# facebookresearch/vector_db_id_compression

Measured on AMD Instinct MI355X. Metric: IDs encoded+decoded / sec (ROC/ANS, bit-exact vs codec.cpp), higher is better.
Workload: dtype u64

## Files before the change

vector_db_id_compression_amd/csrc/roc_u2.h:

```cpp
#pragma once
#include "roc_u.h"
#include "roc_u2_geom.h"

namespace vidc {
namespace dev {

template <int UB>
__device__ __forceinline__ uint32_t u2_word_of(uint32_t x) {
    using U = U2Geom<UB>;
    return (((x >> U::ESH) ^ (U::NE - 1u)) << U::GSH) | ((x >> 6) & (U::G - 1u));
}

__device__ __forceinline__ uint32_t u2_dec_word_of(uint32_t x) { return x >> 6; }

typedef uint4 U2Div;

template <int UB>
__device__ __forceinline__ void u2_build_counts(const uint64_t *bm, uint32_t &E1, v32u &ra, v32u &rb) {
    using U = U2Geom<UB>;
    const uint32_t lane = lane_id();
    uint32_t running = 0;
    E1 = 0;
#pragma unroll
    for (int L1 = 63; L1 >= 0; L1--) {
// ... 137 lines not shown
#else
#define U2P(i) ""
#define U2P_OPERANDS
#endif
#define U2_DIV \
    "v_mul_hi_u32 v36, s58, v7\n"                       \
    "v_mad_u64_u32 v[38:39], s[78:79], s58, v8, v[36:37]\n" \
    "v_mad_u64_u32 v[42:43], s[78:79], s59, v7, v[38:39]\n" \
    "v_mov_b32 v40, v43\n" \
    "v_mad_u64_u32 v[46:47], s[78:79], s59, v8, v[40:41]\n"
#define U2_DIV_REM \
    "v_mul_lo_u32 v48, v46, v9\n" \
    "v_sub_u32 v48, s58, v48\n"
#define U2_INSTALL \
    "v_mov_b32 v7, v54\n v_mov_b32 v8, v55\n v_mov_b32 v10, v56\n v_mov_b32 v11, v57\n" \
    "v_sub_u32 v9, s85, v2\n" \
    "v_max_i32 v9, 1, v9\n" \
    "v_sub_u32 v29, 0, v9\n" \
    "s_sub_u32 s68, s85, 63\n" \
    "v_sub_u32 v58, s68, v2\n" \
    "v_max_i32 v58, 0, v58\n" \
    "v_lshlrev_b32 v58, 4, v58\n" \
    "global_load_dwordx4 v[54:57], v58, s[94:95]\n"
#define U2_ENC_ENTRY \
    "v_sub_u32 v58, s85, v2\n" \
    "v_max_i32 v58, 0, v58\n" \
    "v_lshlrev_b32 v58, 4, v58\n" \
    "global_load_dwordx4 v[54:57], v58, s[94:95]\n" \
    "s_waitcnt vmcnt(0)\n" \
    U2_INSTALL U2_DIV U2_DIV_REM \
    "s_mov_b32 s69, 0\n" \
    "s_min_u32 s70, s86, 63\n"

#define U2_ENC_TOP "1:\n" U2_ENC_TOP_NL
#define U2_ENC_TOP_NL \
    U2P(130) U2P(131) \
    "v_lshrrev_b32_e64 v14, 16, s40\n"                  \
    "v_bfe_u32 v15, s40, 0, 16\n"                       \
    "v_add_u32 v16, v48, v14\n"                         \
    "v_mad_u32_u24 v16, v15, s41, v16\n"                \
    "v_mul_hi_u32 v17, v16, v10\n"                      \
    "v_mad_i32_i24 v18, v17, v29, v16\n"                \
    "v_sub_u32 v19, v18, v9\n" \
    "v_min_u32 v52, v18, v19\n"                         \
    "v_ashrrev_i32 v27, 31, v19\n"                      \
    "v_add3_u32 v20, v17, v27, 1\n"                     \
    "v_readlane_b32 s42, v52, s69\n"                    \
    "v_add_co_u32_e64 v50, s[78:79], v46, v20\n"        \
    "v_addc_co_u32_e64 v51, s[78:79], 0, v47, s[78:79]\n" \
    "v_mov_b32 v12, s42\n" U2P(132) \
    "v_cmp_le_u32 vcc, v4, v12\n"                       \
    "v_lshlrev_b64 v[22:23], s40, 1\n"                  \
    "v_bfi_b32 v24, v22, 0, s66\n" \
    "v_readlane_b32 s50, v50, s69\n" \
    "v_readlane_b32 s51, v51, s69\n" \
    U2P(133) \
    "v_bfi_b32 v25, v23, 0, s67\n" \
    "v_mov_b32 v26, s65\n" \
    "ds_write_b64 v26, v[24:25]\n" \
    "s_ff1_i32_b64 s43, vcc\n" \
    "s_set_gpr_idx_on s43, gpr_idx(SRC0)\n" \
    "v_mov_b32 v13, v64\n"                              \
    "s_set_gpr_idx_off\n" U2P(134) \
    "s_and_b32 m0, s60, 63\n"                           \
    "s_cmp_ge_u32 s51, s73\n" \
    "v_writelane_b32 v5, s50, m0\n" \
// ... 73 lines not shown
    "s_sub_u32 s68, s60, s61\n"                         \
    "s_cmp_ge_u32 s68, 48\n" \
    "s_cselect_b32 s71, 0, s71\n"
#define U2_ENC_BOT(ORDER, LSHR) U2_ENC_BOT_T(ORDER, LSHR, U2_RING_CHECK, "s_cbranch_scc1 1b\n")
#define U2_ENC_BOT_T(ORDER, LSHR, RING, TAIL) \
    "v_mbcnt_lo_u32_b32 v49, s66, 0\n" \
    "v_mbcnt_hi_u32_b32 v49, s67, v49\n" \
    "v_cmp_eq_u32 vcc, v49, v12\n"                      \
    "v_sub_u32 v48, s58, v48\n"                         \
    "s_and_b64 s[82:83], vcc, s[66:67]\n" \
    "s_ff1_i32_b64 s48, s[82:83]\n" \
    "s_or_b32 s40, s46, s48\n"                          U2P(140) \
    "s_mov_b32 m0, s62\n" \
    "s_and_b32 s68, s40, 0xffff\n" \
    "s_or_b32 s68, s68, s54\n" \
    "v_writelane_b32 v5, s68, m0\n"                     \
    ORDER U2P(141) \
    "s_set_gpr_idx_on s43, gpr_idx(DST)\n" \
    "v_mov_b32 v64, v13\n" \
    "s_set_gpr_idx_off\n" U2P(142) \
    LSHR                                                \
    "s_cselect_b32 s71, s70, 0\n" \
    "s_cmp_ge_u32 s59, 0x7ff80000\n" \
    "s_cselect_b32 s71, 0, s71\n" \
    RING \
    "s_add_u32 s69, s69, 1\n" U2P(143) \
    "s_cmp_lt_u32 s69, s71\n" \
    TAIL
#define U2_ENC_ORDER \
    "s_mov_b32 m0, s69\n" \
    "s_lshr_b64 s[98:99], s[58:59], 31\n"              \
    "v_writelane_b32 v6, s40, m0\n"

#define U2_ENC_TOP_D \
    U2P(130) U2P(131) \
    "v_lshrrev_b32_e64 v14, 16, s40\n"                  \
    "v_bfe_u32 v15, s40, 0, 16\n"                       \
    "v_add_u32 v16, v48, v14\n"                         \
    "v_mad_u32_u24 v16, v15, s41, v16\n"                \
    "v_mul_hi_u32 v17, v16, v10\n"                      \
    "v_mad_i32_i24 v18, v17, v29, v16\n"                \
    "v_sub_u32 v19, v18, v9\n" \
    "v_min_u32 v52, v18, v19\n"                         \
    "v_ashrrev_i32 v27, 31, v19\n"                      \
    "v_add3_u32 v20, v17, v27, 1\n"                     \
    "v_readlane_b32 s42, v52, s69\n"                    U2P(132) \
    "v_cmp_ge_u32_e64 s[82:83], s42, v4\n"              \
    "v_add_co_u32_e64 v50, s[78:79], v46, v20\n"        \
    "v_addc_co_u32_e64 v51, s[78:79], 0, v47, s[78:79]\n" \
    "v_readlane_b32 s50, v50, s69\n" \
    "v_readlane_b32 s51, v51, s69\n" \
    U2P(133) \
    "s_ff1_i32_b64 s43, s[82:83]\n" \
    "s_set_gpr_idx_on s43, gpr_idx(SRC0)\n" \
    "v_mov_b32 v13, v64\n"                              \
    "s_set_gpr_idx_off\n" U2P(134) \
    "s_and_b32 m0, s60, 63\n"                           \
    "s_cmp_ge_u32 s51, s73\n" \
    "v_writelane_b32 v5, s50, m0\n" \
    "s_cselect_b32 s52, s51, s50\n" \
    "s_cselect_b32 s53, 0, s51\n" \
    "s_addc_u32 s60, s60, 0\n" \
    "s_lshl_b64 s[54:55], s[52:53], s76\n" \
    "s_and_b32 s62, s60, 63\n"                          \
    "s_cmp_ge_u32 s55, s74\n" \
    "s_cselect_b32 s41, 0, s75\n" \
    "s_cselect_b32 s56, s55, s54\n" \
    "s_cselect_b32 s57, 0, s55\n" \
    "s_addc_u32 s60, s60, 0\n" \
    "s_lshl_b64 s[58:59], s[56:57], s77\n"              U2P(135) \
    "v_readlane_b32 s49, v4, s43\n" \
    "v_add_u32 v27, s49, v13\n"                         \
    "v_cmp_ge_u32 vcc, s42, v27\n"                      \
    "v_mul_hi_u32 v36, s58, v7\n"                       \
    "s_ff1_i32_b64 s44, vcc\n" \
    "s_lshl_b32 s45, s43, 6\n" \
    "s_or_b32 s45, s45, s44\n" U2P(136)
#define U2_ENC_MID_D \
    "v_lshl_add_u32 v28, s45, 5, v3\n" \
    "v_lshlrev_b32_e64 v26, 2, s45\n" \
    "ds_read_u16 v30, v28 offset:2\n" \
    "ds_read_b32 v31, v26 offset:16\n"                  \
    "v_readlane_b32 s63, v27, s44\n"                    \
    "v_cndmask_b32_e64 v59, -1, 0, vcc\n"               \
    "v_add_u32 v13, v13, v59\n"                         \
    "v_cndmask_b32_e64 v59, -1, 0, s[82:83]\n"          \
    "v_add_u32 v4, v4, v59\n"                           U2P(137) \
    "s_sub_u32 s42, s42, s63\n"                         \
    "v_cmp_lt_u32_e64 s[82:83], s42, v60\n"             U2P(138) \
    "v_mad_u64_u32 v[38:39], s[78:79], s58, v8, v[36:37]\n" \
    "v_mad_u64_u32 v[42:43], s[78:79], s59, v7, v[38:39]\n" \
    "v_mov_b32 v40, v43\n" \
    "v_mad_u64_u32 v[46:47], s[78:79], s59, v8, v[40:41]\n" \
    "s_waitcnt lgkmcnt(0)\n" U2P(139)
#define U2_ENC_BOT_D(ORDER, LSHR, RING, TAIL) \
    "v_add_u32 v32, v30, v31\n"                         \
    "v_cndmask_b32_e64 v61, v62, v28, s[82:83]\n"       \
    "v_readlane_b32 s40, v32, s42\n"                    \
    "ds_write_b16 v61, v30\n"                           \
    "v_mul_lo_u32 v48, v46, v9\n"                       \
    "v_sub_u32 v48, s58, v48\n"                         U2P(140) \
    "s_mov_b32 m0, s62\n" \
    "s_and_b32 s68, s40, 0xffff\n" \
    "s_or_b32 s68, s68, s54\n" \
    "v_writelane_b32 v5, s68, m0\n"                     \
    ORDER U2P(141) \
    "s_set_gpr_idx_on s43, gpr_idx(DST)\n" \
    "v_mov_b32 v64, v13\n" \
    "s_set_gpr_idx_off\n" U2P(142) \
    LSHR                                                \
    "s_cselect_b32 s71, s70, 0\n" \
    "s_cmp_ge_u32 s59, 0x7ff80000\n" \
    "s_cselect_b32 s71, 0, s71\n" \
    RING \
    "s_add_u32 s69, s69, 1\n" U2P(143) \
    "s_cmp_lt_u32 s69, s71\n" \
    TAIL

#define U2_ORDER_FLUSH \
    "v_cmp_gt_u32 vcc, s72, v2\n" \
    "v_add_u32 v58, s87, v2\n" \
    "v_lshlrev_b32 v58, 2, v58\n" \
    "s_and_saveexec_b64 s[96:97], vcc\n" \
    "global_store_dword v58, v6, s[88:89]\n" \
    "s_mov_b64 exec, s[96:97]\n" \
    "s_add_u32 s87, s87, s72\n"

#define U2_ENC_OUTER(FLUSH) \
    "s_lshr_b64 s[98:99], s[58:59], 31\n"              \
    "s_cselect_b32 s99, 0, 1\n" \
    "s_cmp_ge_u32 s59, 0x7ff80000\n" \
    "s_cselect_b32 s99, 1, s99\n" \
    "s_sub_u32 s68, s60, s61\n" \
    "s_cmp_lt_u32 s68, 48\n"                            \
    "s_cbranch_scc1 3f\n" \
    "v_subrev_u32 v27, s61, v2\n"                       \
    "v_and_b32 v27, 63, v27\n" \
    "v_add_u32 v58, s61, v27\n" \
    "v_cmp_gt_u32 vcc, 32, v27\n" \
    "v_cmp_gt_u32 s[96:97], s92, v58\n" \
    "v_lshlrev_b32 v58, 2, v58\n" \
    "s_and_b64 vcc, vcc, s[96:97]\n" \
    "s_and_saveexec_b64 s[96:97], vcc\n" \
    "global_store_dword v58, v5, s[90:91]\n" \
    "s_mov_b64 exec, s[96:97]\n" \
    "s_add_u32 s61, s61, 32\n" \
    "s_cmp_gt_u32 s61, s92\n" \
    "s_cselect_b32 s68, 1, 0\n" \
    "s_or_b32 s93, s93, s68\n" \
    "3:\n" \
// ... 104 lines not shown
    const uint32_t p0 = P < 16u ? P : 16u, p1 = P > 16u ? P - 16u : 0u;
    WStack st;
    {
        const uint64_t ao = rfl64(arena_at(a, l));
        ws_init_empty(st, a.arena + ao, rfl((uint32_t)(arena_at(a, l + 1) - ao)), a.mt, VIDC_MT_TABLE);
    }
    uint64_t head = VIDC_RANS_L;
    uint32_t obuf = 0, obase = 0;
    uint32_t *order = WANT_ORDER ? a.perm + off : nullptr;
    const uint32_t T0 = 0x80000000u >> p0, T1 = 0x80000000u >> p1, MULN = 1u << p1;
    const uint32_t l3off = dense ? 2u * lane + (U2Dense::SLOT_OFF - 2u) : U::G == 4u ? (lane & 3u) * 8u : 0u;
    const uint32_t rmlane = lane - 1u < 15u ? lane : 0u, strip = U2Dense::STRIP_OFF + 4u * lane;

#ifdef U2_PROF
    uint32_t prof[14] = {0, 0, 0, 0, 0, 0, 0, 0, 0, 0, 0, 0, 0, 0};
#endif
#ifdef U2_PROF2
    uint64_t prof2[8] = {0, 0, 0, 0, 0, 0, 0, 0};
    prof2[2] = __builtin_readcyclecounter();
#endif
    uint32_t nmax = n;
    while (nmax) {
        if (st.sp - st.lo >= U2_RING_ROOM) ws_spill32(st);
        if (nmax < 3u || u2_needs_generic(head)) {
            const uint32_t x = dense ? u2d_slow_step(head, st, nmax, E1, ra, rb, smem, p0, p1)
                                     : u2_slow_step<UB>(head, st, nmax, E1, ra, rb, bm, p0, p1);
            if (WANT_ORDER) {
                if (lane == 0) order[obase] = x;
                obase++;
            }
            nmax--;
            continue;
        }
        uint32_t s_x = 0, s_mul = 0, s_t = 0, s_waddr = U::BITMAP_BYTES, s_D0 = rfl(nmax), s_left = rfl(nmax - 2u);
        uint64_t s_w = 0, s_B = rfl64(head);
        uint64_t z0 = 0, z1 = 0, z2 = 0;
        uint64_t qh = 0;
        uint32_t rr = 0;
        st.sp = rfl(st.sp);
        st.lo = rfl(st.lo);
        st.err = rfl(st.err);
        obase = rfl(obase);
#ifdef U2_PROF2
        const uint64_t tp0 = __builtin_readcyclecounter();
#endif
#define U2_ENC_ASM(BODY)                                                                                                  \
        asm volatile(BODY                                                                                                 \
            : "+{v4}"(E1), "+{v5}"(st.win), "+{v6}"(obuf), "+{v[64:95]}"(ra), "+{v[96:127]}"(rb),                          \
              "+{v[46:47]}"(qh), "+{v48}"(rr), "+{s40}"(s_x), "+{s41}"(s_mul), "+{s[58:59]}"(s_B), "+{s60}"(st.sp),          \
              "+{s61}"(st.lo), "+{s65}"(s_waddr), "+{s[66:67]}"(s_w), "+{s69}"(s_t), "+{s85}"(s_D0), "+{s86}"(s_left),       \
              "+{s87}"(obase), "+{s93}"(st.err), "+{v[20:21]}"(z0), "+{v[36:37]}"(z1), "+{v[40:41]}"(z2) U2P_OPERANDS       \
            : "{v2}"(lane), "{v3}"(l3off), "{s73}"(T0), "{s74}"(T1), "{s75}"(MULN), "{s76}"(p0), "{s77}"(p1),                \
              "{s[88:89]}"(order), "{s[90:91]}"(st.mem), "{s92}"(st.cap), "{s[94:95]}"(dtab), "{v60}"(rmlane), "{v62}"(strip) \
            : "memory", "vcc", "scc", "v7", "v8", "v9", "v10", "v11", "v12", "v13", "v14", "v15", "v16", "v17", "v18", "v19",  \
              "v22", "v23", "v24", "v25", "v26", "v27", "v28", "v29", "v30", "v31", "v32", "v33", "v34", "v35", "v38", "v39",\
              "v42", "v43", "v44", "v45", "v49", "v50", "v51", "v52", "v54", "v55", "v56", "v57", "v58", "v59", "v61",              \
              "s42", "s43", "s44", "s45", "s46", "s47", "s48", "s49", "s50", "s51", "s52", "s53", "s54", "s55", "s56", "s57",\
              "s62", "s63", "s64", "s68", "s70", "s71", "s72", "s78", "s79", "s80", "s81", "s82", "s83", "s84", "s96",       \
              "s97", "s98", "s99")
        if (dense) {
#define U2_STEP_D(ORDER, LSHR) U2_ENC_TOP_D U2_ENC_MID_D U2_ENC_BOT_D(ORDER, LSHR, "", "s_cbranch_scc0 7f\n")
#define U2_LAST_D(ORDER, LSHR) U2_ENC_TOP_D U2_ENC_MID_D U2_ENC_BOT_D(ORDER, LSHR, U2_RING_CHECK, "s_cbranch_scc1 1b\n")
            if (WANT_ORDER) U2_ENC_ASM(U2_ENC_ENTRY "1:\n" U2_STEP_D(U2_ENC_ORDER, "") U2_STEP_D(U2_ENC_ORDER, "") U2_STEP_D(U2_ENC_ORDER, "") U2_STEP_D(U2_ENC_ORDER, "") U2_STEP_D(U2_ENC_ORDER, "") U2_STEP_D(U2_ENC_ORDER, "") U2_STEP_D(U2_ENC_ORDER, "")
                                       U2_LAST_D(U2_ENC_ORDER, "") "7:\n" U2_ENC_OUTER(U2_ORDER_FLUSH));
            else U2_ENC_ASM(U2_ENC_ENTRY "1:\n" U2_STEP_D("", "s_lshr_b64 s[98:99], s[58:59], 31\n") U2_STEP_D("", "s_lshr_b64 s[98:99], s[58:59], 31\n") U2_STEP_D("", "s_lshr_b64 s[98:99], s[58:59], 31\n")
                            U2_LAST_D("", "s_lshr_b64 s[98:99], s[58:59], 31\n") "7:\n" U2_ENC_OUTER(""));
#undef U2_STEP_D
#undef U2_LAST_D
        } else if (U::G == 4u) {
#define U2_STEP_X(ORDER, LSHR) U2_ENC_TOP_NL U2_ENC_MID_G4 U2_ENC_SLICE1_G4 U2_ENC_L3_G4 U2_ENC_BOT_T(ORDER, LSHR, "", "s_cbranch_scc0 7f\n")
            if (WANT_ORDER) U2_ENC_ASM(U2_ENC_ENTRY "1:\n" U2_STEP_X(U2_ENC_ORDER, "") U2_STEP_X(U2_ENC_ORDER, "") U2_STEP_X(U2_ENC_ORDER, "") U2_STEP_X(U2_ENC_ORDER, "") U2_STEP_X(U2_ENC_ORDER, "") U2_STEP_X(U2_ENC_ORDER, "") U2_STEP_X(U2_ENC_ORDER, "")
                                       U2_ENC_TOP_NL U2_ENC_MID_G4 U2_ENC_SLICE1_G4 U2_ENC_L3_G4 U2_ENC_BOT(U2_ENC_ORDER, "") "7:\n" U2_ENC_OUTER(U2_ORDER_FLUSH));
            else U2_ENC_ASM(U2_ENC_ENTRY "1:\n" U2_STEP_X("", "s_lshr_b64 s[98:99], s[58:59], 31\n") U2_STEP_X("", "s_lshr_b64 s[98:99], s[58:59], 31\n") U2_STEP_X("", "s_lshr_b64 s[98:99], s[58:59], 31\n")
                            U2_ENC_TOP_NL U2_ENC_MID_G4 U2_ENC_SLICE1_G4 U2_ENC_L3_G4 U2_ENC_BOT("", "s_lshr_b64 s[98:99], s[58:59], 31\n") "7:\n" U2_ENC_OUTER(""));
#undef U2_STEP_X
        } else {
#define U2_STEP_X1(ORDER, LSHR) U2_ENC_TOP_NL U2_ENC_MID_G1 U2_ENC_SLICE1("6") U2_ENC_L3_G1 U2_ENC_BOT_T(ORDER, LSHR, "", "s_cbranch_scc0 7f\n")
            if (WANT_ORDER) U2_ENC_ASM(U2_ENC_ENTRY "1:\n" U2_STEP_X1(U2_ENC_ORDER, "") U2_STEP_X1(U2_ENC_ORDER, "") U2_STEP_X1(U2_ENC_ORDER, "") U2_STEP_X1(U2_ENC_ORDER, "") U2_STEP_X1(U2_ENC_ORDER, "") U2_STEP_X1(U2_ENC_ORDER, "") U2_STEP_X1(U2_ENC_ORDER, "")
                                       U2_ENC_TOP_NL U2_ENC_MID_G1 U2_ENC_SLICE1("6") U2_ENC_L3_G1 U2_ENC_BOT(U2_ENC_ORDER, "") "7:\n" U2_ENC_OUTER(U2_ORDER_FLUSH));
            else U2_ENC_ASM(U2_ENC_ENTRY "1:\n" U2_STEP_X1("", "s_lshr_b64 s[98:99], s[58:59], 31\n") U2_STEP_X1("", "s_lshr_b64 s[98:99], s[58:59], 31\n") U2_STEP_X1("", "s_lshr_b64 s[98:99], s[58:59], 31\n")
                            U2_ENC_TOP_NL U2_ENC_MID_G1 U2_ENC_SLICE1("6") U2_ENC_L3_G1 U2_ENC_BOT("", "s_lshr_b64 s[98:99], s[58:59], 31\n") "7:\n" U2_ENC_OUTER(""));
#undef U2_STEP_X1
        }
#undef U2_ENC_ASM
#ifdef U2_PROF2
        prof2[0] += __builtin_readcyclecounter() - tp0;
        prof2[1] += 1;
        prof2[4] += s_t == 63u;
        prof2[5] += st.sp - st.lo >= 62u;
        prof2[6] += u2_needs_generic(s_B);
        prof2[7] += s_t;
#endif
        head = s_B + (uint64_t)((s_x & 0xffffu) * s_mul + (s_x >> 16));
        if (!dense) bm[s_waddr >> 3] = s_w & ~(1ull << (s_x & 63u));
        ws_window(st);
        if (__builtin_expect((head >> 63) != 0ull, 0)) {
            ws_prepare(st);
            ans_u_push(head, st, 0u, 0u);
            ans_u_push(head, st, 0u, 0u);
// ... 298 lines not shown
#define U2_DEC_TOP_L(LA, LB, LC, LD)                    \
    U2PD(130) U2PD(131) \
    "s_and_b32 s46, s58, s73\n"                         \
    "s_lshr_b64 s[58:59], s[58:59], s77\n" \
    "s_lshr_b64 s[98:99], s[58:59], 31\n"              \
    "s_cbranch_scc0 " LA "f\n"                          \
    LB ":\n" \
    "s_and_b32 s40, s58, s74\n"                         \
    "s_lshr_b64 s[58:59], s[58:59], s76\n" \
    "s_lshr_b64 s[98:99], s[58:59], 31\n" \
    "s_cbranch_scc0 " LC "f\n" \
    LD ":\n" \
    "s_pack_ll_b32_b16 s40, s40, s46\n"                 U2PD(132)
#define U2_DEC_IDX_G4 \
    "s_lshr_b32 s45, s40, 8\n"                          \
    "v_lshl_add_u32 v28, s45, 5, v3\n" \
    "v_lshlrev_b32_e64 v29, 2, s45\n"                   \
    "ds_read_b64 v[30:31], v28\n" \
    "ds_read_b32 v29, v29\n"                            \
    "s_bfe_u32 s47, s40, 0x20006\n"                     \
    "s_lshr_b32 s65, s40, 5\n"                          U2PD(133)
#define U2_DEC_IDX_G1 \
    "s_lshr_b32 s45, s40, 6\n" \
    "v_lshl_add_u32 v28, s45, 3, v3\n" \
    "v_lshlrev_b32_e64 v29, 2, s45\n" \
    "ds_read_b64 v[30:31], v28\n" \
    "ds_read_b32 v29, v29\n" \
    "s_lshr_b32 s65, s40, 5\n" U2PD(133)
#define U2_DEC_AFTER_RANK \
    "v_writelane_b32 v6, s40, m0\n"                     \
    "v_ashrrev_i32 v58, 31, v58\n" \
    "v_sub_u32 v4, v4, v58\n"                           U2PD(142)
#ifndef U2_DEC_STEP
#define U2_DEC_STEP 3
#endif
#define U2_DEC_TOP_P(LA, LB) \
    U2PD(130) U2PD(131) \
    "s_lshr_b64 s[98:99], s[58:59], s56\n"             \
    "s_cbranch_scc0 " LA "f\n" \
    "s_and_b32 s46, s58, s73\n"                         \
    "s_bfe_u32 s40, s58, s57\n"                         \
    "s_lshr_b64 s[58:59], s[58:59], s63\n"              \
    "s_lshr_b64 s[98:99], s[58:59], 31\n"              \
    "s_cselect_b32 s59, s59, s58\n"                     \
    "s_cselect_b32 s58, s58, s41\n" \
    "s_addc_u32 s60, s60, -1\n"                         \
    LB ":\n" \
    "s_pack_ll_b32_b16 s40, s40, s46\n"                 U2PD(132)
#define U2_DEC_SIDE_P(LA, LB) \
    LA ":\n"                                            \
    "s_and_b32 s46, s58, s73\n" \
    "s_lshr_b64 s[58:59], s[58:59], s77\n" \
    "s_sub_u32 s60, s60, 1\n" \
    "s_mov_b32 s59, s58\n" \
    "s_mov_b32 s58, s41\n" \
    "s_and_b32 s40, s58, s74\n" \
    "s_lshr_b64 s[58:59], s[58:59], s76\n" \
    "s_branch " LB "b\n"
#if U2_DEC_STEP & 2
#define U2_DEC_W_IDX "s_sub_u32 s42, s60, 1\n"
#define U2_DEC_W_LOAD "v_readlane_b32 s41, v5, s42\n"
#else
#define U2_DEC_W_IDX ""
#define U2_DEC_W_LOAD ""
#endif
#if U2_DEC_STEP & 1
#define U2_DEC_BFM ""
// ... 77 lines not shown
    "ds_read_u16 v29, v29\n"                            \
    "s_lshr_b32 s65, s40, 5\n"                          U2PD(133)
#define U2_DEC_MID_W \
    "s_lshr_b32 s43, s45, 8\n"                          \
    "s_and_b32 s44, s45, 255\n"                         \
    U2_DEC_BFM \
    "s_and_b32 m0, s60, 63\n" U2PD(134) \
    "v_readlane_b32 s62, v10, s69\n"                    \
    "v_readlane_b32 s49, v4, s43\n"                     \
    "v_lshl_add_u32 v38, s43, 9, v11\n"                 \
    "v_lshl_add_u32 v39, s44, 4, v3\n"                  \
    "v_med3_i32 v39, v39, 0, 63\n" \
    "v_writelane_b32 v5, s58, m0\n"                     \
    "v_lshlrev_b64 v[34:35], v39, s[54:55]\n"           \
    "v_and_b32 v35, 0x7fffffff, v35\n"                  U2PD(135) \
    "s_cmp_ge_u32 s59, s62\n" \
    "s_cselect_b32 s50, s59, s58\n" \
    "s_cselect_b32 s51, 0, s59\n" \
    "s_addc_u32 s60, s60, 0\n" U2PD(136) \
    U2_DEC_W_IDX \
    "s_mul_i32 s52, s50, s75\n"                         \
    "s_mul_hi_u32 s53, s50, s75\n" \
    "s_mul_i32 s68, s51, s75\n" \
    "s_add_u32 s53, s53, s68\n" \
    "s_mov_b32 m0, s69\n" U2PD(137)
#define U2_DEC_RANK_W \
    U2_DEC_RANK_1W("32") \
    U2_DEC_W_LOAD                                       \
    U2_DEC_INS_ADDR \
    "v_lshlrev_b32 v27, s40, v12\n"                     \
    "v_writelane_b32 v6, s40, m0\n"                     \
    "ds_or_b32 v26, v27\n"                              \
    "ds_add_u64 v38, v[34:35]\n"                        U2PD(141)
#define U2_DEC_BOT_T_U(RLO, RSPAN)                      \
    "s_sub_u32 s68, s60, s61\n"                         \
    "s_add_u32 s68, s68, " RLO "\n" \
    "s_add_u32 s69, s69, 1\n" \
    "s_add_u32 s75, s75, 1\n" \
    "s_add_u32 s58, s52, s64\n"                         \
    "s_addc_u32 s59, s53, 0\n" \
    "s_cmp_gt_u32 s68, " RSPAN "\n" \
    "s_cselect_b32 s71, 0, s70\n" \
    "s_lshr_b64 s[98:99], s[58:59], 31\n"              \
    "s_cselect_b32 s71, s71, 0\n" U2PD(143) \
    "s_cmp_lt_u32 s69, s71\n"
#define U2_DEC_BOT_NR_U \
    "s_add_u32 s69, s69, 1\n" \
    "s_add_u32 s75, s75, 1\n" \
    "s_add_u32 s58, s52, s64\n"                         \
    "s_addc_u32 s59, s53, 0\n" \
    "s_lshr_b64 s[98:99], s[58:59], 31\n"              \
    "s_cselect_b32 s71, s70, 0\n" U2PD(143) \
    "s_cmp_lt_u32 s69, s71\n"
#if U2_DEC_STEP & 2
#define U2_DEC_TOP_U(LA, LB, LC, LD) U2_DEC_TOP_P(LA, LB)
#define U2_DEC_SIDE_U(LA, LB, LC, LD) U2_DEC_SIDE_P(LA, LB)
#define U2_DEC_ENTRY_U U2_DEC_ENTRY U2_DEC_W_IDX U2_DEC_W_LOAD
#define U2_DEC_OUTER_U(RLO, RSPAN) U2_DEC_OUTER_TR(RLO, RSPAN, U2_DEC_W_IDX U2_DEC_W_LOAD)
#else
#define U2_DEC_TOP_U(LA, LB, LC, LD) U2_DEC_TOP_L(LA, LB, LC, LD)
#define U2_DEC_SIDE_U(LA, LB, LC, LD) U2_DEC_SIDE(LA, LB, LC, LD)
#define U2_DEC_ENTRY_U U2_DEC_ENTRY
#define U2_DEC_OUTER_U(RLO, RSPAN) U2_DEC_OUTER_T(RLO, RSPAN)
#endif
#define U2_DEC_STEP_U(IDX, MID, RANK, LA, LB, LC, LD) U2_DEC_TOP_U(LA, LB, LC, LD) IDX MID RANK U2_DEC_BOT_NR_U "s_cbranch_scc0 2f\n"
#define U2_DEC_LOOP8_U(IDX, MID, RANK) \
// ... 182 lines not shown
    const uint32_t M1 = (1u << p1) - 1u, M0 = (1u << p0) - 1u;
    const uint32_t pop_thr = 31u + p1, pop_bfe = (p0 << 16) | p1, pop_sh = p1 + p0;
    uint64_t *out = a.out + ooff;
    wave_sync();
#ifdef U2_PROF
    uint32_t prof[14] = {0, 0, 0, 0, 0, 0, 0, 0, 0, 0, 0, 0, 0, 0};
#endif

#ifdef U2_PROF2
    uint32_t dbg[4] = {0, 0, 0, 0};
#define U2_DBG(k) dbg[k]++
#else
#define U2_DBG(k)
#endif
    uint32_t i = 0;
    constexpr uint32_t RING_LO = U2_DEC_RING_LO, RING_HI = U2_DEC_RING_HI;
    while (i < n) {
        {
            const uint32_t res = st.sp - st.lo;
            if (res > 56u) ws_spill32(st);
            else if (res < 22u && st.lo != 0u) ws_refill32(st);
        }
        if (lt_2p31(head) || st.sp - st.lo < RING_LO || st.sp - st.lo > RING_HI) {
            U2_DBG(0);
            uint32_t x;
            if constexpr (WORD) x = u2w_slow_dec_step(head, st, i + 1u, E1, smem, p0, p1);
            else x = u2_slow_dec_step<UB>(head, st, i + 1u, E1, rows, bm, p0, p1);
            if (lane == 0) out[n - 1u - i] = (uint64_t)x;
            i++;
            continue;
        }
        U2_DBG(1);
        uint32_t s_t = 0, s_N0 = rfl(i + 1u), s_left = rfl(n - i), s_oidx = rfl(n - 1u - i);
        uint64_t s_h = rfl64(head), oring = 0;
        st.sp = rfl(st.sp);
        st.lo = rfl(st.lo);
#define U2_DEC_IN_W "{v12}"(ins_bit), "{s[54:55]}"(field_ones),
#define U2_DEC_ASM(BODY, ...)                                                                                             \
        asm volatile(BODY                                                                                                 \
            : "+{v4}"(E1), "+{v5}"(st.win), "+{v[6:7]}"(oring),                                                           \
              "+{s[58:59]}"(s_h), "+{s60}"(st.sp), "+{s69}"(s_t), "+{s85}"(s_N0), "+{s86}"(s_left), "+{s87}"(s_oidx)        \
              U2P_OPERANDS                                                                                                 \
            : __VA_ARGS__ "{v2}"(lane), "{v3}"(l3off), "{v8}"(ins_mul), "{v9}"(ins_add), "{v11}"(row_lane), "{s61}"(st.lo), \
              "{s73}"(M1), "{s74}"(M0), "{s76}"(p0), "{s77}"(p1), "{s[88:89]}"(out), "{s[94:95]}"(dtab),                    \
              "{s56}"(pop_thr), "{s57}"(pop_bfe), "{s63}"(pop_sh)                                                            \
            : "memory", "vcc", "scc", "v10", "v26", "v27", "v28", "v29", "v30", "v31", "v32", "v33", "v34", "v35", "v36",     \
              "v37", "v38", "v39", "v54", "v55", "v56", "v57", "v58", "s40", "s41", "s42", "s43", "s44", "s45", "s46", "s47", \
              "s49", "s50", "s51", "s52", "s53", "s62", "s64", "s65", "s66", "s67", "s68", "s70", "s71", "s72", "s75", "s96", \
              "s97", "s98", "s99" U2PD_CLOBBERS)
        if constexpr (WORD) U2_DEC_ASM(U2_DEC_ENTRY_U U2_DEC_LOOP8_U(U2_DEC_IDX_W, U2_DEC_MID_W, U2_DEC_RANK_W) U2_DEC_OUTER_U("-18", "35"), U2_DEC_IN_W);
        else if (U::G == 4u) U2_DEC_ASM(U2_DEC_ENTRY_U U2_DEC_LOOP8_U(U2_DEC_IDX_G4, U2_DEC_MID_U, U2_DEC_RANK_U_G4) U2_DEC_OUTER_U("-18", "35"));
        else U2_DEC_ASM(U2_DEC_ENTRY_U U2_DEC_LOOP8_U(U2_DEC_IDX_G1, U2_DEC_MID_U1, U2_DEC_RANK_U_G1) U2_DEC_OUTER_U("-18", "35"));
#undef U2_DEC_ASM
#undef U2_DEC_IN_W
        head = s_h;
        ws_window(st);
        if (__builtin_expect(lt_2p31(head), 0)) {
            ws_prepare(st);
            head = (uint64_t)ws_pop(st) | (head << 32);
        }
        i = s_N0 + s_t - 1u;
    }
    uint32_t bits = 0;
    for (uint32_t w = lane; w < U::BITMAP_BYTES / 8u; w += 64) bits += popc64(bm[w]);
#pragma unroll
    for (int o = 32; o > 0; o >>= 1) bits += (uint32_t)__shfl_xor((int)bits, o, 64);
#ifdef U2_PROF2
    if (lane == 0) { a.slots[0] = dbg[0]; a.slots[1] = dbg[1]; a.slots[2] = rfl(bits); a.slots[3] = n; }
#endif
#ifdef U2_PROF
    if (lane == 0)
        for (int q = 0; q < 14; q++) a.slots[q] = prof[q];
#endif
    if (rfl(bits) != n) {
        wave_sync();
        roc_decode_u_body<UB>(a, smem);
        return;
    }
    if (lane == 0) {
        const bool clean = (head == VIDC_RANS_L) && (st.sp == st.draws - draws0);
        a.end_state[l] = clean ? 0u : 1u;
        a.status[l] = st.err ? ((st.err & 1u) ? VIDC_ST_OVERFLOW : VIDC_ST_MT) : VIDC_ST_OK;
    }
// ... 318 lines not shown
```

Baseline: 61.44 million.

## Add classified fast-path renormalization for dense encode and word decode loops

Restructures the dense encoder step so the common case, where the head needs no renormalization (checked by one shift against 63-P), does a single combined shift and skips both slice compare/select sequences. Renormalizing steps branch to out-of-line side blocks. In the word decoder it adds a classified loop (enabled by raising U2_DEC_STEP to 7) that decodes both slices with one combined shift and branches out only for the rare refill or spill cases, limiting block length where the classification stays valid. A host-side reference header models the classified math for validation. The cost is extra branches and code size, plus a risk to bit-exactness in the rare paths.

Result: faster. 65.52 million (median of 6 runs) (+6.6%).

```diff
diff --git a/vector_db_id_compression_amd/csrc/roc_u2.h b/vector_db_id_compression_amd/csrc/roc_u2.h
--- a/vector_db_id_compression_amd/csrc/roc_u2.h
+++ b/vector_db_id_compression_amd/csrc/roc_u2.h
@@ -193,6 +193,9 @@
     "s_mov_b32 s69, 0\n" \
     "s_min_u32 s70, s86, 63\n"
 
+#ifndef U2_ENC_STEP
+#define U2_ENC_STEP 1
+#endif
 #define U2_ENC_TOP "1:\n" U2_ENC_TOP_NL
 #define U2_ENC_TOP_NL \
     U2P(130) U2P(131) \
@@ -332,7 +335,7 @@
     "s_lshr_b64 s[98:99], s[58:59], 31\n"              \
     "v_writelane_b32 v6, s40, m0\n"
 
-#define U2_ENC_TOP_D \
+#define U2_ENC_TOP_D_A \
     U2P(130) U2P(131) \
     "v_lshrrev_b32_e64 v14, 16, s40\n"                  \
     "v_bfe_u32 v15, s40, 0, 16\n"                       \
@@ -354,7 +357,8 @@
     "s_ff1_i32_b64 s43, s[82:83]\n" \
     "s_set_gpr_idx_on s43, gpr_idx(SRC0)\n" \
     "v_mov_b32 v13, v64\n"                              \
-    "s_set_gpr_idx_off\n" U2P(134) \
+    "s_set_gpr_idx_off\n" U2P(134)
+#define U2_ENC_SLICES_D(MULSEL) \
     "s_and_b32 m0, s60, 63\n"                           \
     "s_cmp_ge_u32 s51, s73\n" \
     "v_writelane_b32 v5, s50, m0\n" \
@@ -364,11 +368,12 @@
     "s_lshl_b64 s[54:55], s[52:53], s76\n" \
     "s_and_b32 s62, s60, 63\n"                          \
     "s_cmp_ge_u32 s55, s74\n" \
-    "s_cselect_b32 s41, 0, s75\n" \
+    MULSEL \
     "s_cselect_b32 s56, s55, s54\n" \
     "s_cselect_b32 s57, 0, s55\n" \
     "s_addc_u32 s60, s60, 0\n" \
-    "s_lshl_b64 s[58:59], s[56:57], s77\n"              U2P(135) \
+    "s_lshl_b64 s[58:59], s[56:57], s77\n"
+#define U2_ENC_TOP_D_B \
     "v_readlane_b32 s49, v4, s43\n" \
     "v_add_u32 v27, s49, v13\n"                         \
     "v_cmp_ge_u32 vcc, s42, v27\n"                      \
@@ -376,6 +381,7 @@
     "s_ff1_i32_b64 s44, vcc\n" \
     "s_lshl_b32 s45, s43, 6\n" \
     "s_or_b32 s45, s45, s44\n" U2P(136)
+#define U2_ENC_TOP_D U2_ENC_TOP_D_A U2_ENC_SLICES_D("s_cselect_b32 s41, 0, s75\n") U2P(135) U2_ENC_TOP_D_B
 #define U2_ENC_MID_D \
     "v_lshl_add_u32 v28, s45, 5, v3\n" \
     "v_lshlrev_b32_e64 v26, 2, s45\n" \
@@ -393,18 +399,19 @@
     "v_mov_b32 v40, v43\n" \
     "v_mad_u64_u32 v[46:47], s[78:79], s59, v8, v[40:41]\n" \
     "s_waitcnt lgkmcnt(0)\n" U2P(139)
-#define U2_ENC_BOT_D(ORDER, LSHR, RING, TAIL) \
+#define U2_ENC_BOT_D_A \
     "v_add_u32 v32, v30, v31\n"                         \
     "v_cndmask_b32_e64 v61, v62, v28, s[82:83]\n"       \
     "v_readlane_b32 s40, v32, s42\n"                    \
     "ds_write_b16 v61, v30\n"                           \
     "v_mul_lo_u32 v48, v46, v9\n"                       \
-    "v_sub_u32 v48, s58, v48\n"                         U2P(140) \
+    "v_sub_u32 v48, s58, v48\n"                         U2P(140)
+#define U2_ENC_BOT_D_W \
     "s_mov_b32 m0, s62\n" \
     "s_and_b32 s68, s40, 0xffff\n" \
     "s_or_b32 s68, s68, s54\n" \
-    "v_writelane_b32 v5, s68, m0\n"                     \
-    ORDER U2P(141) \
+    "v_writelane_b32 v5, s68, m0\n"
+#define U2_ENC_BOT_D_C(LSHR, RING, TAIL) \
     "s_set_gpr_idx_on s43, gpr_idx(DST)\n" \
     "v_mov_b32 v64, v13\n" \
     "s_set_gpr_idx_off\n" U2P(142) \
@@ -416,6 +423,23 @@
     "s_add_u32 s69, s69, 1\n" U2P(143) \
     "s_cmp_lt_u32 s69, s71\n" \
     TAIL
+#define U2_ENC_BOT_D(ORDER, LSHR, RING, TAIL) U2_ENC_BOT_D_A U2_ENC_BOT_D_W ORDER U2P(141) U2_ENC_BOT_D_C(LSHR, RING, TAIL)
+
+#define U2_ENC_CLASS_D(LS) \
+    "s_lshr_b64 s[52:53], s[50:51], s39\n"             \
+    "s_cbranch_scc1 " LS "f\n" \
+    "s_lshl_b64 s[58:59], s[50:51], s38\n"
+#define U2_ENC_STEP_DC(LT, LS, ORDER, LSHR, RING, TAIL) \
+    LT ":\n" U2_ENC_TOP_D_A U2_ENC_CLASS_D(LS) U2P(135) U2_ENC_TOP_D_B U2_ENC_MID_D U2_ENC_BOT_D_A ORDER U2P(141) U2_ENC_BOT_D_C(LSHR, RING, TAIL)
+#define U2_ENC_SIDE_DC(LS, LNEXT, ORDER_S, RING) \
+    LS ":\n" U2_ENC_SLICES_D("s_cselect_b32 s64, 0xffff0000, -1\n") U2P(135) U2_ENC_TOP_D_B U2_ENC_MID_D U2_ENC_BOT_D_A U2_ENC_BOT_D_W ORDER_S U2P(141) \
+    U2_ENC_BOT_D_C("s_lshr_b64 s[98:99], s[58:59], 31\n", RING, "s_cbranch_scc1 " LNEXT "b\n s_branch 7f\n")
+#define U2_ENC_ORDER_S \
+    "s_mov_b32 m0, s69\n" \
+    "s_and_b32 s68, s40, s64\n"                         \
+    "v_writelane_b32 v6, s40, m0\n" \
+    "s_mov_b32 s40, s68\n"
+#define U2_ENC_NOORDER_S "s_and_b32 s40, s40, s64\n"
 
 #define U2_ORDER_FLUSH \
     "v_cmp_gt_u32 vcc, s72, v2\n" \
@@ -586,11 +610,12 @@
             nmax--;
             continue;
         }
-        uint32_t s_x = 0, s_mul = 0, s_t = 0, s_waddr = U::BITMAP_BYTES, s_D0 = rfl(nmax), s_left = rfl(nmax - 2u);
+        uint32_t s_x = 0, s_mul = rfl(MULN), s_t = 0, s_waddr = U::BITMAP_BYTES, s_D0 = rfl(nmax), s_left = rfl(nmax - 2u);
         uint64_t s_w = 0, s_B = rfl64(head);
         uint64_t z0 = 0, z1 = 0, z2 = 0;
         uint64_t qh = 0;
         uint32_t rr = 0;
+        const uint32_t s_P = rfl(P), s_PR = rfl(63u - P);
         st.sp = rfl(st.sp);
         st.lo = rfl(st.lo);
         st.err = rfl(st.err);
@@ -605,7 +630,8 @@
               "+{s61}"(st.lo), "+{s65}"(s_waddr), "+{s[66:67]}"(s_w), "+{s69}"(s_t), "+{s85}"(s_D0), "+{s86}"(s_left),       \
               "+{s87}"(obase), "+{s93}"(st.err), "+{v[20:21]}"(z0), "+{v[36:37]}"(z1), "+{v[40:41]}"(z2) U2P_OPERANDS       \
             : "{v2}"(lane), "{v3}"(l3off), "{s73}"(T0), "{s74}"(T1), "{s75}"(MULN), "{s76}"(p0), "{s77}"(p1),                \
-              "{s[88:89]}"(order), "{s[90:91]}"(st.mem), "{s92}"(st.cap), "{s[94:95]}"(dtab), "{v60}"(rmlane), "{v62}"(strip) \
+              "{s[88:89]}"(order), "{s[90:91]}"(st.mem), "{s92}"(st.cap), "{s[94:95]}"(dtab), "{v60}"(rmlane), "{v62}"(strip), \
+              "{s38}"(s_P), "{s39}"(s_PR)                                                                                    \
             : "memory", "vcc", "scc", "v7", "v8", "v9", "v10", "v11", "v12", "v13", "v14", "v15", "v16", "v17", "v18", "v19",  \
               "v22", "v23", "v24", "v25", "v26", "v27", "v28", "v29", "v30", "v31", "v32", "v33", "v34", "v35", "v38", "v39",\
               "v42", "v43", "v44", "v45", "v49", "v50", "v51", "v52", "v54", "v55", "v56", "v57", "v58", "v59", "v61",              \
@@ -613,12 +639,27 @@
               "s62", "s63", "s64", "s68", "s70", "s71", "s72", "s78", "s79", "s80", "s81", "s82", "s83", "s84", "s96",       \
               "s97", "s98", "s99")
         if (dense) {
+#if U2_ENC_STEP & 1
+#define U2_STEP_D(LT, LS, ORDER, LSHR) U2_ENC_STEP_DC(LT, LS, ORDER, LSHR, "", "s_cbranch_scc0 7f\n")
+#define U2_LAST_D(LT, LS, ORDER, LSHR) U2_ENC_STEP_DC(LT, LS, ORDER, LSHR, U2_RING_CHECK, "s_cbranch_scc1 1b\n s_branch 7f\n")
+#define U2_L31 "s_lshr_b64 s[98:99], s[58:59], 31\n"
+            if (WANT_ORDER) U2_ENC_ASM(U2_ENC_ENTRY "1:\n" U2_STEP_D("110", "120", U2_ENC_ORDER, "") U2_STEP_D("111", "121", U2_ENC_ORDER, "") U2_STEP_D("112", "122", U2_ENC_ORDER, "") U2_STEP_D("113", "123", U2_ENC_ORDER, "")
+                                       U2_STEP_D("114", "124", U2_ENC_ORDER, "") U2_STEP_D("115", "125", U2_ENC_ORDER, "") U2_STEP_D("116", "126", U2_ENC_ORDER, "") U2_LAST_D("117", "127", U2_ENC_ORDER, "")
+                                       U2_ENC_SIDE_DC("120", "111", U2_ENC_ORDER_S, "") U2_ENC_SIDE_DC("121", "112", U2_ENC_ORDER_S, "") U2_ENC_SIDE_DC("122", "113", U2_ENC_ORDER_S, "") U2_ENC_SIDE_DC("123", "114", U2_ENC_ORDER_S, "")
+                                       U2_ENC_SIDE_DC("124", "115", U2_ENC_ORDER_S, "") U2_ENC_SIDE_DC("125", "116", U2_ENC_ORDER_S, "") U2_ENC_SIDE_DC("126", "117", U2_ENC_ORDER_S, "") U2_ENC_SIDE_DC("127", "110", U2_ENC_ORDER_S, U2_RING_CHECK)
+                                       "7:\n" U2_ENC_OUTER(U2_ORDER_FLUSH));
+            else U2_ENC_ASM(U2_ENC_ENTRY "1:\n" U2_STEP_D("110", "120", "", U2_L31) U2_STEP_D("111", "121", "", U2_L31) U2_STEP_D("112", "122", "", U2_L31) U2_LAST_D("113", "123", "", U2_L31)
+                            U2_ENC_SIDE_DC("120", "111", U2_ENC_NOORDER_S, "") U2_ENC_SIDE_DC("121", "112", U2_ENC_NOORDER_S, "") U2_ENC_SIDE_DC("122", "113", U2_ENC_NOORDER_S, "") U2_ENC_SIDE_DC("123", "110", U2_ENC_NOORDER_S, U2_RING_CHECK)
+                            "7:\n" U2_ENC_OUTER(""));
+#undef U2_L31
+#else
 #define U2_STEP_D(ORDER, LSHR) U2_ENC_TOP_D U2_ENC_MID_D U2_ENC_BOT_D(ORDER, LSHR, "", "s_cbranch_scc0 7f\n")
 #define U2_LAST_D(ORDER, LSHR) U2_ENC_TOP_D U2_ENC_MID_D U2_ENC_BOT_D(ORDER, LSHR, U2_RING_CHECK, "s_cbranch_scc1 1b\n")
             if (WANT_ORDER) U2_ENC_ASM(U2_ENC_ENTRY "1:\n" U2_STEP_D(U2_ENC_ORDER, "") U2_STEP_D(U2_ENC_ORDER, "") U2_STEP_D(U2_ENC_ORDER, "") U2_STEP_D(U2_ENC_ORDER, "") U2_STEP_D(U2_ENC_ORDER, "") U2_STEP_D(U2_ENC_ORDER, "") U2_STEP_D(U2_ENC_ORDER, "")
                                        U2_LAST_D(U2_ENC_ORDER, "") "7:\n" U2_ENC_OUTER(U2_ORDER_FLUSH));
             else U2_ENC_ASM(U2_ENC_ENTRY "1:\n" U2_STEP_D("", "s_lshr_b64 s[98:99], s[58:59], 31\n") U2_STEP_D("", "s_lshr_b64 s[98:99], s[58:59], 31\n") U2_STEP_D("", "s_lshr_b64 s[98:99], s[58:59], 31\n")
                             U2_LAST_D("", "s_lshr_b64 s[98:99], s[58:59], 31\n") "7:\n" U2_ENC_OUTER(""));
+#endif
 #undef U2_STEP_D
 #undef U2_LAST_D
         } else if (U::G == 4u) {
@@ -983,7 +1024,7 @@
     "v_ashrrev_i32 v58, 31, v58\n" \
     "v_sub_u32 v4, v4, v58\n"                           U2PD(142)
 #ifndef U2_DEC_STEP
-#define U2_DEC_STEP 3
+#define U2_DEC_STEP 7
 #endif
 #define U2_DEC_TOP_P(LA, LB) \
     U2PD(130) U2PD(131) \
@@ -1127,6 +1168,82 @@
     "v_writelane_b32 v6, s40, m0\n"                     \
     "ds_or_b32 v26, v27\n"                              \
     "ds_add_u64 v38, v[34:35]\n"                        U2PD(141)
+#define U2_DEC_TOP_C(LA, LB, LD) \
+    U2PD(130) U2PD(131) \
+    "s_and_b32 s46, s58, s73\n"                         \
+    "s_bfe_u32 s40, s58, s57\n"                         \
+    "s_lshr_b64 s[50:51], s[58:59], s63\n"              \
+    "s_sub_u32 s98, s50, s62\n" \
+    "s_subb_u32 s99, s51, 0\n"                          \
+    "s_cbranch_scc1 " LA "f\n" \
+    "s_cmp_ge_u32 s51, s62\n"                           \
+    "s_cbranch_scc1 " LD "f\n" \
+    LB ":\n" \
+    "s_pack_ll_b32_b16 s40, s40, s46\n"                 U2PD(132)
+#define U2_DEC_SIDE_C(LA, LB, LD, LS) \
+    LA ":\n" \
+    "s_sub_u32 s60, s60, 1\n"                           \
+    "s_lshr_b64 s[98:99], s[58:59], s56\n"              \
+    "v_readlane_b32 s41, v5, s60\n"                     \
+    "s_cbranch_scc0 " LS "f\n" \
+    "s_mov_b32 s51, s50\n"                              \
+    "s_mov_b32 s50, s41\n" \
+    "s_branch " LB "b\n" \
+    LS ":\n"                                            \
+    "s_lshr_b64 s[50:51], s[58:59], s77\n" \
+    "s_mov_b32 s51, s50\n" \
+    "s_mov_b32 s50, s41\n" \
+    "s_and_b32 s40, s50, s74\n"                         \
+    "s_lshr_b64 s[50:51], s[50:51], s76\n" \
+    "s_cmp_ge_u32 s51, s62\n"                           \
+    "s_cbranch_scc0 " LB "b\n" \
+    "s_and_b32 m0, s60, 63\n" \
+    "s_add_u32 s60, s60, 1\n" \
+    "v_writelane_b32 v5, s50, m0\n" \
+    "s_mov_b32 s50, s51\n" \
+    "s_mov_b32 s51, 0\n" \
+    "s_branch " LB "b\n" \
+    LD ":\n"                                            \
+    "s_and_b32 m0, s60, 63\n" \
+    "s_add_u32 s60, s60, 1\n" \
+    "v_writelane_b32 v5, s50, m0\n" \
+    "s_mov_b32 s50, s51\n" \
+    "s_mov_b32 s51, 0\n" \
+    "s_branch " LB "b\n"
+#define U2_DEC_MID_WC \
+    "s_lshr_b32 s43, s45, 8\n"                          \
+    "s_and_b32 s44, s45, 255\n"                         \
+    "s_add_u32 s42, s69, 1\n"                           U2PD(134) \
+    "v_readlane_b32 s49, v4, s43\n"                     \
+    "v_lshl_add_u32 v38, s43, 9, v11\n"                 \
+    "v_lshl_add_u32 v39, s44, 4, v3\n"                  \
+    "v_med3_i32 v39, v39, 0, 63\n" \
+    "v_lshlrev_b64 v[34:35], v39, s[54:55]\n"           \
+    "v_and_b32 v35, 0x7fffffff, v35\n"                  U2PD(135) U2PD(136) \
+    "s_mul_i32 s52, s50, s75\n"                         \
+    "s_mul_hi_u32 s53, s50, s75\n" \
+    "s_mul_i32 s68, s51, s75\n" \
+    "s_add_u32 s53, s53, s68\n" \
+    "s_mov_b32 m0, s69\n" U2PD(137)
+#define U2_DEC_RANK_WC \
+    U2_DEC_RANK_1W("32") \
+    "v_readlane_b32 s62, v10, s42\n"                    \
+    U2_DEC_INS_ADDR \
+    "v_lshlrev_b32 v27, s40, v12\n"                     \
+    "v_writelane_b32 v6, s40, m0\n"                     \
+    "ds_or_b32 v26, v27\n"                              \
+    "ds_add_u64 v38, v[34:35]\n"                        U2PD(141)
+#define U2_DEC_LQ_LOAD "v_readlane_b32 s62, v10, s69\n"
+#define U2_DEC_ENTRY_C U2_DEC_ENTRY U2_DEC_LQ_LOAD
+#define U2_DEC_OUTER_C(RLO, RSPAN) U2_DEC_OUTER_TR(RLO, RSPAN, U2_DEC_LQ_LOAD)
+#define U2_DEC_STEP_C(LA, LB, LD) U2_DEC_TOP_C(LA, LB, LD) U2_DEC_IDX_W U2_DEC_MID_WC U2_DEC_RANK_WC U2_DEC_BOT_NR_U "s_cbranch_scc0 2f\n"
+#define U2_DEC_LOOP8_C \
+    "1:\n" U2_DEC_STEP_C("20", "21", "22") U2_DEC_STEP_C("30", "31", "32") U2_DEC_STEP_C("40", "41", "42") U2_DEC_STEP_C("50", "51", "52") \
+    U2_DEC_STEP_C("60", "61", "62") U2_DEC_STEP_C("70", "71", "72") U2_DEC_STEP_C("80", "81", "82") \
+    U2_DEC_TOP_C("90", "91", "92") U2_DEC_IDX_W U2_DEC_MID_WC U2_DEC_RANK_WC U2_DEC_BOT_T_U("-18", "35") "s_cbranch_scc1 1b\n s_branch 2f\n" \
+    U2_DEC_SIDE_C("20", "21", "22", "23") U2_DEC_SIDE_C("30", "31", "32", "33") U2_DEC_SIDE_C("40", "41", "42", "43") \
+    U2_DEC_SIDE_C("50", "51", "52", "53") U2_DEC_SIDE_C("60", "61", "62", "63") U2_DEC_SIDE_C("70", "71", "72", "73") \
+    U2_DEC_SIDE_C("80", "81", "82", "83") U2_DEC_SIDE_C("90", "91", "92", "93") "2:\n"
 #define U2_DEC_BOT_T_U(RLO, RSPAN)                      \
     "s_sub_u32 s68, s60, s61\n"                         \
     "s_add_u32 s68, s68, " RLO "\n" \
@@ -1375,6 +1492,10 @@
         }
         U2_DBG(1);
         uint32_t s_t = 0, s_N0 = rfl(i + 1u), s_left = rfl(n - i), s_oidx = rfl(n - 1u - i);
+#if U2_DEC_STEP & 4
+        const bool classified = rfl((uint32_t)(WORD && (p1 == 0u || i + 1u <= (1u << p0)))) != 0u;
+        s_left = rfl(classified && p1 != 0u ? min(n - i, (1u << p0) - i) : n - i);
+#endif
         uint64_t s_h = rfl64(head), oring = 0;
         st.sp = rfl(st.sp);
         st.lo = rfl(st.lo);
@@ -1391,7 +1512,14 @@
               "v37", "v38", "v39", "v54", "v55", "v56", "v57", "v58", "s40", "s41", "s42", "s43", "s44", "s45", "s46", "s47", \
               "s49", "s50", "s51", "s52", "s53", "s62", "s64", "s65", "s66", "s67", "s68", "s70", "s71", "s72", "s75", "s96", \
               "s97", "s98", "s99" U2PD_CLOBBERS)
+#if U2_DEC_STEP & 4
+        if constexpr (WORD) {
+            if (classified) U2_DEC_ASM(U2_DEC_ENTRY_C U2_DEC_LOOP8_C U2_DEC_OUTER_C("-18", "35"), U2_DEC_IN_W);
+            else U2_DEC_ASM(U2_DEC_ENTRY_U U2_DEC_LOOP8_U(U2_DEC_IDX_W, U2_DEC_MID_W, U2_DEC_RANK_W) U2_DEC_OUTER_U("-18", "35"), U2_DEC_IN_W);
+        }
+#else
         if constexpr (WORD) U2_DEC_ASM(U2_DEC_ENTRY_U U2_DEC_LOOP8_U(U2_DEC_IDX_W, U2_DEC_MID_W, U2_DEC_RANK_W) U2_DEC_OUTER_U("-18", "35"), U2_DEC_IN_W);
+#endif
         else if (U::G == 4u) U2_DEC_ASM(U2_DEC_ENTRY_U U2_DEC_LOOP8_U(U2_DEC_IDX_G4, U2_DEC_MID_U, U2_DEC_RANK_U_G4) U2_DEC_OUTER_U("-18", "35"));
         else U2_DEC_ASM(U2_DEC_ENTRY_U U2_DEC_LOOP8_U(U2_DEC_IDX_G1, U2_DEC_MID_U1, U2_DEC_RANK_U_G1) U2_DEC_OUTER_U("-18", "35"));
 #undef U2_DEC_ASM
diff --git a/vector_db_id_compression_amd/csrc/u2_renorm_ref.h b/vector_db_id_compression_amd/csrc/u2_renorm_ref.h
--- /dev/null
+++ b/vector_db_id_compression_amd/csrc/u2_renorm_ref.h
@@ -0,0 +1,133 @@
+#pragma once
+#include <stdint.h>
+
+namespace vidc {
+
+enum U2RenormClass : uint32_t {
+    U2_ENC_NONE = 0, U2_ENC_SLICE0 = 1, U2_ENC_SLICE1 = 2, U2_ENC_BOTH = 3,
+    U2_DEC_COMMON = 0, U2_DEC_UNDONE = 1, U2_DEC_A = 2, U2_DEC_SLICE1 = 3, U2_DEC_D = 4, U2_DEC_SLICE1_SPILL = 5, U2_DEC_OTHER = 6
+};
+
+inline uint32_t u2_rn_p0(uint32_t P) { return P < 16u ? P : 16u; }
+inline uint32_t u2_rn_p1(uint32_t P) { return P > 16u ? (P - 16u > 16u ? 16u : P - 16u) : 0u; }
+
+struct U2EncStep {
+    uint64_t head;
+    uint32_t nwords;
+    uint32_t words[2];
+    uint32_t cls;
+};
+
+inline U2EncStep u2_enc_two(uint64_t q, uint32_t x, uint32_t p0, uint32_t p1) {
+    U2EncStep r{0, 0, {0, 0}, U2_ENC_NONE};
+    uint64_t head = q;
+    if (head >= ((0x80000000ull >> p0) << 32)) { r.words[r.nwords++] = (uint32_t)head; head >>= 32; r.cls |= U2_ENC_SLICE0; }
+    head = (head << p0) + (uint64_t)(x & 0xffffu);
+    if (head >= ((0x80000000ull >> p1) << 32)) { r.words[r.nwords++] = (uint32_t)head; head >>= 32; r.cls |= U2_ENC_SLICE1; }
+    head = (head << p1) + (uint64_t)(x >> 16);
+    r.head = head;
+    return r;
+}
+
+inline U2EncStep u2_enc_classified(uint64_t q, uint32_t x, uint32_t p0, uint32_t p1) {
+    U2EncStep r{0, 0, {0, 0}, U2_ENC_NONE};
+    const uint32_t P = p0 + p1, mul = 1u << p1;
+    uint64_t B;
+    uint32_t xs = x;
+    if ((q >> (63u - P)) == 0ull) {
+        B = q << P;
+    } else {
+        const uint32_t T0 = 0x80000000u >> p0, T1 = 0x80000000u >> p1;
+        const uint32_t q_lo = (uint32_t)q, q_hi = (uint32_t)(q >> 32);
+        uint32_t ring[2] = {0, 0}, sp = 0;
+        ring[sp] = q_lo;
+        const bool s0 = q_hi >= T0;
+        const uint64_t a = s0 ? (uint64_t)q_hi : q;
+        sp += s0 ? 1u : 0u;
+        const uint64_t A = a << p0;
+        const uint32_t slot = sp;
+        const bool s1 = (uint32_t)(A >> 32) >= T1;
+        const uint32_t mask = s1 ? 0xffff0000u : 0xffffffffu;
+        const uint64_t b = s1 ? (A >> 32) : A;
+        sp += s1 ? 1u : 0u;
+        B = b << p1;
+        if (slot < 2u) ring[slot] = (x & 0xffffu) | (uint32_t)A;
+        xs = x & mask;
+        r.nwords = sp;
+        r.words[0] = ring[0];
+        r.words[1] = ring[1];
+        r.cls = (s0 ? U2_ENC_SLICE0 : 0u) | (s1 ? U2_ENC_SLICE1 : 0u);
+    }
+    r.head = B + (uint64_t)((xs & 0xffffu) * mul + (xs >> 16));
+    if (r.nwords < 2u) r.words[1] = 0;
+    if (r.nwords < 1u) r.words[0] = 0;
+    return r;
+}
+
+struct U2DecStep {
+    uint64_t H;
+    uint32_t x;
+    int32_t delta;
+    uint32_t top;
+    uint32_t cls;
+};
+
+inline U2DecStep u2_dec_two(uint64_t head, uint32_t w0, uint32_t w1, uint32_t p0, uint32_t p1, uint32_t nmax) {
+    const uint64_t lq = 0x80000000ull / nmax;
+    U2DecStep r{0, 0, 0, 0, U2_DEC_COMMON};
+    uint32_t popped = 0;
+    const uint32_t wv[2] = {w0, w1};
+    bool r1 = false, r0 = false, sp = false;
+    const uint32_t x_hi = (uint32_t)(head & ((1ull << p1) - 1ull));
+    head >>= p1;
+    if (head < 0x80000000ull) { head = (head << 32) | wv[popped++]; r1 = true; }
+    const uint32_t x_lo = (uint32_t)(head & ((1ull << p0) - 1ull));
+    head >>= p0;
+    if (head < 0x80000000ull) { head = (head << 32) | wv[popped++]; r0 = true; }
+    r.delta = -(int32_t)popped;
+    if (head >= (lq << 32)) { r.top = (uint32_t)head; head >>= 32; r.delta++; sp = true; }
+    r.H = head;
+    r.x = (x_hi << 16) | x_lo;
+    r.cls = r1 && r0 ? U2_DEC_OTHER : r1 ? (sp ? U2_DEC_SLICE1_SPILL : U2_DEC_SLICE1) : r0 ? (sp ? U2_DEC_UNDONE : U2_DEC_A) : sp ? U2_DEC_D : U2_DEC_COMMON;
+    return r;
+}
+
+inline bool u2_dec_block_valid(uint32_t nmax_last, uint32_t p0, uint32_t p1) { return p1 == 0u || nmax_last <= (1u << p0); }
+
+inline U2DecStep u2_dec_classified(uint64_t head, uint32_t w0, uint32_t p0, uint32_t p1, uint32_t nmax) {
+    const uint32_t lq = 0x80000000u / nmax;
+    const uint32_t lo = (uint32_t)head;
+    const uint32_t m1 = (1u << p1) - 1u, m0 = (1u << p0) - 1u;
+    U2DecStep r{0, 0, 0, 0, U2_DEC_COMMON};
+    const uint32_t x_hi = lo & m1;
+    uint32_t x_lo = (lo >> p1) & m0;
+    const uint64_t h = head >> (p1 + p0);
+    if (h < (uint64_t)lq) {
+        if ((head >> (31u + p1)) != 0ull) {
+            r.H = (h << 32) | w0;
+            r.delta = -1;
+            r.cls = U2_DEC_A;
+        } else {
+            uint64_t t = (((head >> p1) & 0xffffffffull) << 32) | w0;
+            x_lo = w0 & m0;
+            t >>= p0;
+            r.delta = -1;
+            r.cls = U2_DEC_SLICE1;
+            if ((uint32_t)(t >> 32) >= lq) { r.top = (uint32_t)t; t >>= 32; r.delta = 0; r.cls = U2_DEC_SLICE1_SPILL; }
+            r.H = t;
+        }
+    } else if ((uint32_t)(h >> 32) >= lq) {
+        r.top = (uint32_t)h;
+        r.H = h >> 32;
+        r.delta = 1;
+        r.cls = U2_DEC_D;
+    } else {
+        r.H = h;
+        r.cls = h < 0x80000000ull ? U2_DEC_UNDONE : U2_DEC_COMMON;
+        r.top = h < 0x80000000ull ? w0 : 0u;
+    }
+    r.x = (x_hi << 16) | x_lo;
+    return r;
+}
+
+}
```
